# OSU-NLP-Group/saev

Hardware: AMD Instinct MI355X
Metric: activations/sec (train step), d_in=1024 x32 k=32 (higher is better)
Workload: dtype f32 (encoder: fp16 MFMA first pass with a rigorous error margin, survivors recomputed exactly in fp32; all else fp32)

## Files before the change

### saev_amd/csrc/common.h

```cpp
#pragma once
#include <hip/hip_runtime.h>
#include <stdint.h>

#define WAVE 64

typedef float f32x4 __attribute__((ext_vector_type(4)));
typedef float f32x16 __attribute__((ext_vector_type(16)));

__device__ __forceinline__ int32_t f2key(float f) {
    int32_t b = __float_as_int(f);
    return b >= 0 ? b : (b ^ 0x7fffffff);
}
__device__ __forceinline__ float key2f(int32_t k) {
    return __int_as_float(k >= 0 ? k : (k ^ 0x7fffffff));
}
__device__ __forceinline__ uint32_t f2ukey(float f) {
    uint32_t b = __float_as_uint(f);
    return (b & 0x80000000u) ? ~b : (b | 0x80000000u);
}
__device__ __forceinline__ float ukey2f(uint32_t k) {
    return __uint_as_float((k & 0x80000000u) ? (k & 0x7fffffffu) : ~k);
}

__device__ __forceinline__ float wave_sum(float v) {
#pragma unroll
    for (int o = 32; o > 0; o >>= 1) v += __shfl_xor(v, o, 64);
    return v;
}
__device__ __forceinline__ double wave_sum_d(double v) {
#pragma unroll
    for (int o = 32; o > 0; o >>= 1) v += __shfl_xor(v, o, 64);
    return v;
}
__device__ __forceinline__ int wave_sum_i(int v) {
#pragma unroll
    for (int o = 32; o > 0; o >>= 1) v += __shfl_xor(v, o, 64);
    return v;
}
__device__ __forceinline__ float wave_max(float v) {
#pragma unroll
    for (int o = 32; o > 0; o >>= 1) v = fmaxf(v, __shfl_xor(v, o, 64));
    return v;
}

#define NEG_INF (-__builtin_huge_valf())

__device__ __forceinline__ float rpg_apply(float g, float sc, float w) { return __builtin_fmaf(-sc, w, g); }
template <int NV>
__device__ __forceinline__ float rpg_row_stats(const f32x4 (&g)[NV], const f32x4 (&w)[NV], int project, float* sc_out) {
    float dot = 0.f, nsq = 0.f;
#pragma unroll
    for (int n = 0; n < NV; ++n)
#pragma unroll
        for (int e = 0; e < 4; ++e) { dot = __builtin_fmaf(g[n][e], w[n][e], dot); nsq = __builtin_fmaf(w[n][e], w[n][e], nsq); }
    dot = wave_sum(dot);
    nsq = wave_sum(nsq);
    const float sc = (project && nsq > 0.f) ? dot / nsq : 0.f;
    float sq = 0.f;
#pragma unroll
    for (int n = 0; n < NV; ++n)
#pragma unroll
        for (int e = 0; e < 4; ++e) { const float t = rpg_apply(g[n][e], sc, w[n][e]); sq = __builtin_fmaf(t, t, sq); }
    *sc_out = sc;
    return wave_sum(sq);
}
```

### saev_amd/csrc/kernels.h

```cpp
#pragma once
#include <hip/hip_runtime.h>
#include <stdint.h>

#include "../../include/saev_amd.h"

enum { EPI_DENSE = 0, EPI_TOPK = 1 };

struct EncodeArgs {
    const float* x;
    const float* W_enc;
    const float* b_enc;
    int n_rows, D, S;
    int s_splits;
    float* h_out;
    int ngroups;
    int32_t* gmax;
    int gmax_stride;
    int32_t* cand_cnt;
    float* cand_val;
    int32_t* cand_idx;
    int cand_cap;
    int cand_stride;
    const int32_t* enable_flag;
    int enable_when;
};

size_t encode_gemm_smem_bytes();
hipError_t launch_encode_gemm(const EncodeArgs& a, int epi, hipStream_t stream);
int encode_gemm_tile_rows();
int encode_gemm_tile_latents();

struct SelectDenseArgs {
    const float* h;
    int n_rows, S;
    int k;
    const int32_t* k_dev;
    const int32_t* mask;
    int32_t* idx_out;
    float* val_out;
    int out_stride;
    const int32_t* enable_flag;
    int enable_when;
};
hipError_t launch_select_dense(const SelectDenseArgs& a, hipStream_t stream);

struct SelectCandArgs {
    const int32_t* cand_cnt;
    const float* cand_val;
    const int32_t* cand_idx;
    int cand_cap, cand_stride, n_rows, k;
    int32_t* idx_out;
    float* val_out;
    int out_stride;
    const int32_t* enable_flag;
    int enable_when;
    const float* row_margin;
    const float* x;
    const float* W_encT;
    const float* b_enc;
    int D;
    int32_t* surv_idx;
    float* surv_val;
    int32_t* surv_cnt;
    int32_t* refine_overflow;
    const int32_t* tau_max;
    int32_t* invalid;
    int32_t* ovf;
    int32_t* surv_rng;
    int lat_range, n_ranges;
    const float* sum_part;
    const float* sum_bias;
    int sum_n;
    size_t sum_plane;
};
hipError_t launch_refine_exact(const SelectCandArgs& a, hipStream_t stream);
constexpr int REFINE_CAP = 512;
constexpr int RS_SLICE = 32;
constexpr int RS_ROWS_MAX = 8;
constexpr int RS_LAT_RANGE = 32768;
constexpr int RS_MAX_RANGES = 8;
struct RefineSlicesArgs {
    const int32_t* surv_idx; const int32_t* surv_cnt; float* surv_val; const int32_t* surv_rng;
    const float* xS; const float* WeS; const float* b_enc; float* part;
    int n_rows, S, D, lat_range, n_ranges;
    const int32_t* enable_flag; int enable_when;
};
hipError_t launch_refine_slices(const RefineSlicesArgs& a, hipStream_t stream);
hipError_t launch_select_cand(const SelectCandArgs& a, hipStream_t stream);
hipError_t launch_init_i32(int32_t* p, int32_t v, int n, hipStream_t stream);
hipError_t launch_encoder_init(int32_t* cand_cnt, int n_rows, int32_t* gmax, int n_gmax, hipStream_t stream,
                               int32_t* tau_max = nullptr, const int32_t* enable_flag = nullptr, int enable_when = 0);
hipError_t launch_pre_encode(int32_t* cand_cnt, int n_rows, int32_t* gmax, int n_gmax, const float* xnorm, int D,
                             const float* wg_part, int n_part, const float* scales, int32_t* pre_flag, float* wmax_prev,
                             float* margin, int32_t* flags1, hipStream_t stream);
hipError_t launch_heur_gate(float* state, const int32_t* pre_flag, int32_t* gate, hipStream_t stream);
hipError_t launch_heur_update(float* state, const int32_t* bad, const float* cand_mean, int k, const int32_t* gate,
                              hipStream_t stream);
hipError_t launch_step_zero(saev_step_stats* stats, float* upper, int32_t* flag0, hipStream_t stream);
hipError_t launch_wnorm_max(const float* W_encT, int S, int D, float* wg_scratch, float* wmax, hipStream_t stream);
hipError_t launch_f16r_scales(const float* xmax_part, int n_part, const float* wmax, float* scales, hipStream_t stream);
hipError_t launch_pow2_scale(const float* absmax, float* pair, hipStream_t stream);
hipError_t launch_center_stats(const float* x, const float* mu, int n, int D, float* xnorm, float* wg_absmax,
                               hipStream_t stream, const float* xmax = nullptr);
hipError_t launch_row_margins(const float* xnorm, int n, int D, const float* wg_part, int n_part, const float* scales,
                              int32_t* pre_flag, float* wmax_prev, float* margin, hipStream_t stream);
hipError_t launch_overflow_check(const int32_t* cand_cnt, int n_rows, int cap, const int32_t* pre_flag,
                                 int32_t* need_dense, int32_t* n_overflow, int32_t* cand_max, hipStream_t stream,
                                 int32_t* dense_out = nullptr, int32_t* run_out = nullptr, float* cand_mean = nullptr,
                                 const int32_t* enable_flag = nullptr, const int32_t* dense_src = nullptr);

struct __attribute__((aligned(8))) RowStats {
    float sse_scaled;
    float l0;
    float l1;
    float aux_sse;
    double sse64;
    double sumsq64;
};

struct DecodeArgs {
    const float* x;
    const int32_t* idx;
    const float* val;
    int code_stride, k;
    const float* W_dec;
    const float* b_dec;
    int n_rows, D, S;
    int idx_limit;
    const float* upper;
    float gscale;
    int training;
    float* g;
    float* x_hat;
    int32_t* fired;
    RowStats* rowstats;
    float* gS;
    float* xS;
    float* dval_out;
    uint32_t* csc_bitmap;
    int csc_words;
};
hipError_t launch_decode(const DecodeArgs& a, hipStream_t stream);
bool decode_forms_dval(int D, int k);
bool decode_matry_forms_dval(int D, int k);

constexpr int MAX_PREFIXES = 16;
struct MatryArgs {
    int P;
    int32_t cuts[MAX_PREFIXES];
    float* G;
    int g_rows_all;
};
hipError_t launch_decode_matry(const DecodeArgs& a, const MatryArgs& m, hipStream_t stream);

struct CscArgs {
    const int32_t* idx;
    int code_stride, k;
    const int32_t* k_dev;
    int n_rows, S;
    uint32_t* bitmap;
    int words;
    int32_t* grp_prefix;
    int32_t* counts;
    int32_t* scan_totals;
    int32_t* starts;
    int2* pairs;
    int32_t* chunk_starts;
    int32_t* part_starts;
    int32_t* work_latent;
    int2* pv;
    int32_t* plat;
    const float* val;
    int2* pv2;
    const float* dval;
    int P;
    int32_t cuts[16];
    int32_t* zero_word;
    int32_t epoch;
};
hipError_t launch_csc_build(const CscArgs& a, hipStream_t stream, bool bitmap_clean = false, const float* colsum_m = nullptr,
                            int colsum_D = 0, long colsum_row_stride = 0, float* colsum_partials = nullptr,
                            float* colsum_out = nullptr, bool prefilled = false);

constexpr int DW_CHUNK = 64;

struct DwRowsArgs {
    const int32_t* starts;
    const int32_t* chunk_starts;
    const int32_t* work_latent;
    const int32_t* part_starts;
    const int2* pairs;
    const float* val;
    const float* W_dec;
    const float* g;
    const float* x;
    int D, S;
    int P;
    int32_t cuts[MAX_PREFIXES];
    const int32_t* k_dev;
    int accumulate;
    float* dW_dec;
    float* dW_encT;
    float* db_enc;
    float* partials;
    float* db_partials;
    int lat_lo, lat_hi;
    int part;
    float* dval;
    float2* row_proj;
    int project;
    float* enc_sq;
    uint32_t* clear_bitmap;
    int clear_words;
};
hipError_t launch_dw_rows(const DwRowsArgs& a, int max_work, hipStream_t stream);

constexpr int DWS_RUN = 64, DWS_SLICE = 32;
constexpr int DWS_FIRST = 1, DWS_LAST = 2, DWS_END = 4;
struct DwSlicesArgs {
    const int32_t* starts;
    const int2* pv;
    int2* pv2;
    const int32_t* plat;
    const float* gS;
    const float* xS;
    const float* W_dec;
    int n_rows, D, S, pair_cap;
    int P;
    float* dvp;
    float* dW_dec;
    float* dW_encT;
// ... 325 lines not shown
```

### saev_amd/csrc/select.hip

```cpp
#include "common.h"
#include "kernels.h"

namespace {

constexpr int SD_THREADS = 256;

__device__ __forceinline__ int block_excl_scan_256(int v, int* lds_wave_tot, int& total) {
    const int lane = threadIdx.x & 63, w = threadIdx.x >> 6;
    int incl = v;
#pragma unroll
    for (int o = 1; o < 64; o <<= 1) {
        int n = __shfl_up(incl, o, 64);
        if (lane >= o) incl += n;
    }
    if (lane == 63) lds_wave_tot[w] = incl;
    __syncthreads();
    int base = 0, tot = 0;
#pragma unroll
    for (int i = 0; i < 4; ++i) {
        const int t = lds_wave_tot[i];
        if (i < w) base += t;
        tot += t;
    }
    total = tot;
// ... 327 lines not shown
        int32_t idx = 0x7fffffff;
        if (p < n) { key = f2ukey(cv[p]); idx = ci[p]; }
        const bool sel = p < n && ((key > T) || (key == T && idx <= idx_cut));
        const unsigned long long m = __ballot(sel);
        const int pos = base + __popcll(m & ((1ull << lane) - 1ull));
        if (sel && pos < 64) { s_idx[w][pos] = idx; s_val[w][pos] = ukey2f(key); }
        base += __popcll(m);
    }
    sort_by_idx_and_store(a, row, k, s_idx[w][lane], s_val[w][lane], lane);
}

__device__ __forceinline__ void select_small_row(const SelectCandArgs& a, int row, int n, const float* cv, const int32_t* ci) {
    const int lane = threadIdx.x & 63;
    const int k = min(a.k, n);
    uint32_t key = 0u;
    int32_t idx = 0x7fffffff;
    if (lane < n) {
        key = f2ukey(cv[lane]);
        idx = ci[lane];
    }
#pragma unroll
    for (int size = 2; size <= 64; size <<= 1) {
#pragma unroll
        for (int stride = size >> 1; stride > 0; stride >>= 1) {
            const uint32_t o_key = __shfl_xor(key, stride, 64);
            const int32_t o_idx = __shfl_xor(idx, stride, 64);
            const bool other_first = (o_key > key) || (o_key == key && o_idx < idx);
            const bool up = ((lane & size) == 0);
            const bool lower = ((lane & stride) == 0);
            const bool take_other = (lower == up) ? other_first : !other_first;
            if (take_other) { key = o_key; idx = o_idx; }
        }
    }
    if (a.tau_max != nullptr) {
        const float kth = ukey2f(__shfl(key, max(k - 1, 0), 64));
        if (lane == 0 && (n < a.k || kth < key2f(a.tau_max[row]))) *a.invalid = 1;
    }
    const bool win = lane < k;
    sort_by_idx_and_store(a, row, k, win ? idx : 0x7fffffff, win ? ukey2f(key) : 0.f, lane);
}

template <bool BIG>
__global__ __launch_bounds__(256) void select_cand_kernel(SelectCandArgs a) {
    if (a.enable_flag != nullptr && (*a.enable_flag != 0) != (a.enable_when != 0)) return;
    __shared__ int32_t s_idx[4][64];
    __shared__ float s_val[4][64];
    const int row = blockIdx.x * 4 + (threadIdx.x >> 6);
    if (row >= a.n_rows) return;
    const int cnt = a.cand_cnt[row];
    if (a.ovf != nullptr && (threadIdx.x & 63) == 0 && cnt > a.cand_cap) atomicOr(&a.ovf[0], 1);
    if (a.ovf != nullptr && a.row_margin != nullptr && (threadIdx.x & 63) == 0 && !(a.row_margin[row] < 3.0e38f)) atomicOr(&a.ovf[0], 1);
    const int n = min(cnt, a.cand_cap);
    const float* cv = a.cand_val + (size_t)row * a.cand_stride;
    const int32_t* ci = a.cand_idx + (size_t)row * a.cand_stride;
    __shared__ float l_sum[4][REFINE_CAP];
    if (a.sum_part != nullptr) {
        float* const lv = l_sum[threadIdx.x >> 6];
        for (int j = threadIdx.x & 63; j < n; j += 64) {
            const size_t o = (size_t)row * a.cand_stride + j;
            float sv = 0.f;
            int c = 0;
            for (; c + 8 <= a.sum_n; c += 8) {
                float v[8];
#pragma unroll
                for (int u = 0; u < 8; ++u) v[u] = a.sum_part[(size_t)(c + u) * a.sum_plane + o];
#pragma unroll
                for (int u = 0; u < 8; ++u) sv += v[u];
            }
            for (; c < a.sum_n; ++c) sv += a.sum_part[(size_t)c * a.sum_plane + o];
            lv[j] = sv + a.sum_bias[ci[j]];
        }
        __asm__ volatile("" ::: "memory");
        cv = lv;
    }
    if (n <= 64 && a.row_margin == nullptr) select_small_row(a, row, n, cv, ci);
    else if (n <= 512) select_cand_row<8>(a, row, n, s_idx, s_val, cv, ci);
    else if (n <= 1024) select_cand_row<16>(a, row, n, s_idx, s_val, cv, ci);
    else if (n <= 2048) select_cand_row<32>(a, row, n, s_idx, s_val, cv, ci);
    else if constexpr (BIG) select_cand_row<64>(a, row, n, s_idx, s_val, cv, ci);
    else select_cand_row_stream(a, row, n, s_idx, s_val, cv, ci);
}

__global__ void init_i32_kernel(int32_t* p, int32_t v, int n) {
    const int i = blockIdx.x * blockDim.x + threadIdx.x;
    if (i < n) p[i] = v;
}

__global__ void encoder_init_kernel(int32_t* cand_cnt, int n_rows, int32_t* gmax, int n_gmax, int32_t* tau_max,
                                    const int32_t* enable_flag, int enable_when) {
    if (enable_flag != nullptr && (*enable_flag != 0) != (enable_when != 0)) return;
    const int i = blockIdx.x * blockDim.x + threadIdx.x;
    if (i < n_rows) cand_cnt[i] = 0;
    if (i < n_gmax) gmax[i] = INT32_MIN;
    if (tau_max != nullptr && i < n_rows) tau_max[i] = INT32_MIN;
}
__global__ void step_zero_kernel(saev_step_stats* stats, float* upper, int32_t* flag0) {
    if (threadIdx.x == 0) {
        *stats = saev_step_stats{};
        *upper = 0.f;
        *flag0 = 0;
    }
}

template <int NV>
__global__ __launch_bounds__(256) void refine_exact_kernel(SelectCandArgs a) {
    if (a.enable_flag != nullptr && (*a.enable_flag != 0) != (a.enable_when != 0)) return;
    const int lane = threadIdx.x & 63;
    const int row = blockIdx.x * 4 + (threadIdx.x >> 6);
    if (row >= a.n_rows) return;
    const int ns = a.surv_cnt[row];
    const int D4 = a.D >> 2;
    f32x4 xv[NV];
    const f32x4* xr = reinterpret_cast<const f32x4*>(a.x + (size_t)row * a.D);
#pragma unroll
    for (int n = 0; n < NV; ++n) xv[n] = (lane + 64 * n < D4) ? xr[lane + 64 * n] : f32x4{0.f, 0.f, 0.f, 0.f};
    const int32_t* si = a.surv_idx + (size_t)row * REFINE_CAP;
    float* sv = a.surv_val + (size_t)row * REFINE_CAP;
    for (int j0 = 0; j0 < ns; j0 += 8) {
        const int32_t my = si[min(j0 + (lane & 7), ns - 1)];
        float p[8];
#pragma unroll
        for (int t = 0; t < 8; ++t) {
            const int32_t li = __shfl(my, t, 64);
            const f32x4* wr = reinterpret_cast<const f32x4*>(a.W_encT + (size_t)li * a.D);
            float acc = 0.f;
#pragma unroll
            for (int n = 0; n < NV; ++n) {
                if (lane + 64 * n < D4) {
                    const f32x4 wv = wr[lane + 64 * n];
                    acc += xv[n][0] * wv[0] + xv[n][1] * wv[1] + xv[n][2] * wv[2] + xv[n][3] * wv[3];
                }
            }
            p[t] = acc;
        }
        const float r = wave_reduce_scatter8(p, lane);
        if ((lane & 7) == 0) {
            const int t = lane >> 3;
            if (j0 + t < ns) sv[j0 + t] = r + a.b_enc[si[j0 + t]];
        }
    }
}

typedef int i32x4 __attribute__((ext_vector_type(4)));
__device__ __forceinline__ f32x4 rs_buf_load16(__amdgpu_buffer_rsrc_t r, uint32_t voff) {
    const i32x4 v = __builtin_amdgcn_raw_buffer_load_b128(r, voff, 0, 0);
    return f32x4{__int_as_float(v[0]), __int_as_float(v[1]), __int_as_float(v[2]), __int_as_float(v[3])};
}
__device__ __forceinline__ float group8_reduce_scatter(float (&p)[8], int li) {
    {
        const bool up = (li & 4) != 0;
#pragma unroll
        for (int i = 0; i < 4; ++i) {
            const float keep = up ? p[i + 4] : p[i], send = up ? p[i] : p[i + 4];
            p[i] = keep + __shfl_xor(send, 4, 64);
        }
    }
    {
        const bool up = (li & 2) != 0;
#pragma unroll
        for (int i = 0; i < 2; ++i) {
            const float keep = up ? p[i + 2] : p[i], send = up ? p[i] : p[i + 2];
            p[i] = keep + __shfl_xor(send, 2, 64);
        }
    }
    const bool up = (li & 1) != 0;
    const float keep = up ? p[1] : p[0], send = up ? p[0] : p[1];
    return keep + __shfl_xor(send, 1, 64);
}
#ifndef RS_BATCHES
#define RS_BATCHES 2
#endif
template <int RS_ROWS>
__global__ __launch_bounds__(256) void refine_slices_kernel(RefineSlicesArgs a, int wg_per_combo) {
    if (a.enable_flag != nullptr && (*a.enable_flag != 0) != (a.enable_when != 0)) return;
    const int lane = threadIdx.x & 63, gi = lane >> 3, li = lane & 7;
    const int xcd = blockIdx.x & 7, q = blockIdx.x >> 3;
    const int combo = q / wg_per_combo;
    const int slice = xcd + 8 * (combo / a.n_ranges), range = combo % a.n_ranges;
    if (slice * RS_SLICE >= a.D) return;
    const int wgi = q % wg_per_combo;
    const int lat_lo = range * a.lat_range, lat_hi = min(a.S, lat_lo + a.lat_range);
    const int sel = (lane & 56) << 2;
    const __amdgpu_buffer_rsrc_t wres = __builtin_amdgcn_make_buffer_rsrc(
        const_cast<float*>(a.WeS) + (size_t)slice * a.S * RS_SLICE, 0, (uint32_t)a.S * 128u, 0x00020000);
    const f32x4* const xs = reinterpret_cast<const f32x4*>(a.xS + (size_t)slice * a.n_rows * RS_SLICE);
    float* const part = a.part + (size_t)slice * a.n_rows * REFINE_CAP;
    const uint32_t li16 = (uint32_t)li * 16u;
    const int row0 = (wgi * RS_ROWS * 4 + (int)(threadIdx.x >> 6)) * 8 + gi;
    int jb[RS_ROWS], je[RS_ROWS];
    f32x4 xr[RS_ROWS];
#pragma unroll
    for (int t = 0; t < RS_ROWS; ++t) {
        const int row = row0 + 32 * t;
        const bool rok = row < a.n_rows;
        je[t] = rok ? a.surv_rng[(size_t)row * RS_MAX_RANGES + range] : 0;
        jb[t] = (rok && range > 0) ? a.surv_rng[(size_t)row * RS_MAX_RANGES + range - 1] : 0;
        xr[t] = rok ? xs[(size_t)row * 8 + li] : f32x4{0.f, 0.f, 0.f, 0.f};
    }
    int t = 0, j0 = jb[0], j_end = je[0];
    f32x4 x4 = xr[0];
    auto advance = [&]() {
#pragma unroll
        for (int s = 1; s < RS_ROWS; ++s) {
            const bool adv = j0 >= j_end && t == s - 1;
            t = adv ? s : t;
            j0 = adv ? jb[s] : j0;
            j_end = adv ? je[s] : j_end;
#pragma unroll
            for (int e = 0; e < 4; ++e) x4[e] = adv ? xr[s][e] : x4[e];
        }
    };
    advance();
#pragma unroll 1
    while (__any(j0 < j_end)) {
        const int row = row0 + 32 * t;
        int32_t my[RS_BATCHES];
        bool mine[RS_BATCHES];
        f32x4 w[RS_BATCHES][8];
#pragma unroll
        for (int h = 0; h < RS_BATCHES; ++h) {
            my[h] = (j0 + 8 * h + li < j_end) ? a.surv_idx[(size_t)row * REFINE_CAP + j0 + 8 * h + li] : -1;
            mine[h] = my[h] >= lat_lo && my[h] < lat_hi;
        }
#pragma unroll
        for (int h = 0; h < RS_BATCHES; ++h) {
            const uint32_t off_my = mine[h] ? (uint32_t)my[h] * 128u : 0xFFFFFF00u;
#pragma unroll
            for (int u = 0; u < 8; ++u) {
                const uint32_t off = (uint32_t)__builtin_amdgcn_ds_bpermute(sel + 4 * u, (int)off_my);
                w[h][u] = rs_buf_load16(wres, off | li16);
            }
        }
#pragma unroll
        for (int h = 0; h < RS_BATCHES; ++h) {
            float p[8];
#pragma unroll
            for (int u = 0; u < 8; ++u) p[u] = x4[0] * w[h][u][0] + x4[1] * w[h][u][1] + x4[2] * w[h][u][2] + x4[3] * w[h][u][3];
            const float r = group8_reduce_scatter(p, li);
            if (mine[h]) part[(size_t)row * REFINE_CAP + j0 + 8 * h + li] = r;
        }
        j0 += 8 * RS_BATCHES;
        advance();
    }
}

__global__ __launch_bounds__(256) void rownorm_wgmax_kernel(const float* m, int R, int D, float* wg_max) {
    __shared__ float sh[4];
    const int lane = threadIdx.x & 63, w = threadIdx.x >> 6;
    const int r = blockIdx.x * 4 + w;
    float s = 0.f;
    if (r < R) {
        const f32x4* p = reinterpret_cast<const f32x4*>(m + (size_t)r * D);
        for (int q = lane; q < (D >> 2); q += 64) {
            const f32x4 v = p[q];
            s += v[0] * v[0] + v[1] * v[1] + v[2] * v[2] + v[3] * v[3];
        }
        s = wave_sum(s);
    }
    if (lane == 0) sh[w] = sqrtf(s);
    __syncthreads();
    if (threadIdx.x == 0) wg_max[blockIdx.x] = fmaxf(fmaxf(sh[0], sh[1]), fmaxf(sh[2], sh[3]));
}
__global__ __launch_bounds__(1024) void max_reduce_kernel(const float* v, int n, float* out) {
    __shared__ float sh[16];
    float m = 0.f;
    for (int i = threadIdx.x; i < n; i += 1024) m = fmaxf(m, v[i]);
    m = wave_max(m);
    if ((threadIdx.x & 63) == 0) sh[threadIdx.x >> 6] = m;
    __syncthreads();
    if (threadIdx.x == 0) {
        float t = 0.f;
        for (int i = 0; i < 16; ++i) t = fmaxf(t, sh[i]);
        *out = t;
    }
}
__device__ __forceinline__ float round_f16_sig(float v) {
    const uint32_t b = __float_as_uint(v);
    return __uint_as_float((b + 0x0FFFu + ((b >> 13) & 1u)) & 0xFFFFE000u);
}
__global__ __launch_bounds__(256) void center_stats_kernel(const float* x, const float* mu, int n, int D,
                                                           float* xnorm, float* wg_max, const float* xmax) {
    __shared__ float sh[4];
    const int lane = threadIdx.x & 63, w = threadIdx.x >> 6;
    const int r = blockIdx.x * 4 + w;
    float s = 0.f, m = 0.f, sd = 0.f;
    const float up = xmax != nullptr ? *xmax : 1.0f;
    const float back = (up > 0.f && up < 3.0e38f) ? up : 1.0f, inv = 1.0f / back;
    if (r < n) {
        const f32x4* p = reinterpret_cast<const f32x4*>(x + (size_t)r * D);
        const f32x4* mu4 = reinterpret_cast<const f32x4*>(mu);
        const int nq = D >> 2;
        for (int q0 = lane; q0 < nq; q0 += 256) {
            f32x4 v[4];
#pragma unroll
            for (int u = 0; u < 4; ++u) {
                const int q = q0 + 64 * u;
                v[u] = q < nq ? p[q] - mu4[q] : f32x4{0.f, 0.f, 0.f, 0.f};
            }
#pragma unroll
            for (int u = 0; u < 4; ++u) {
                m = fmaxf(fmaxf(fmaxf(m, fabsf(v[u][0])), fabsf(v[u][1])), fmaxf(fabsf(v[u][2]), fabsf(v[u][3])));
                f32x4 d;
#pragma unroll
                for (int e = 0; e < 4; ++e) d[e] = (v[u][e] - round_f16_sig(v[u][e])) * inv;
                v[u] = v[u] * inv;
                s += v[u][0] * v[u][0] + v[u][1] * v[u][1] + v[u][2] * v[u][2] + v[u][3] * v[u][3];
                sd += d[0] * d[0] + d[1] * d[1] + d[2] * d[2] + d[3] * d[3];
            }
        }
        s = wave_sum(s);
        sd = wave_sum(sd);
        if (lane == 0) { xnorm[2 * r] = back * sqrtf(s); xnorm[2 * r + 1] = back * sqrtf(sd) * 1.000001f; }
    }
    m = wave_max(m);
    if (lane == 0) sh[w] = m;
    __syncthreads();
    if (threadIdx.x == 0) wg_max[blockIdx.x] = fmaxf(fmaxf(sh[0], sh[1]), fmaxf(sh[2], sh[3]));
}
__device__ __forceinline__ float f16r_margin(float xnorm_row, float xdelta_row, float wmax, float dwmax, float bmax, int D, float x_scale) {
    const float rnd = 1.02f * (xdelta_row * wmax + xnorm_row * dwmax + xdelta_row * dwmax);
    const float acc = (1.05f * (float)D * 2.384185791015625e-07f + 7.62939453125e-06f) * xnorm_row * wmax;
    const float sub = sqrtf((float)D) * 6.103515625e-05f / x_scale * wmax;
    const float m = 2.0f * (rnd + acc + sub) + 2.0f * 1.1920929e-07f * bmax;
    return m == m ? m : __builtin_inff();
}
__device__ __forceinline__ bool f16r_scale_ok(float wmax, float w_scale) {
    const float t = wmax * w_scale;
    return t < 60000.0f && (t >= 2048.0f || wmax == 0.f);
}
__global__ __launch_bounds__(256) void row_margin_kernel(const float* xnorm, int n, int D, const float* wg_part, int n_part,
                                                         const float* scales, int32_t* pre_flag, float* wmax_prev,
                                                         float* margin) {
    __shared__ float sh[3][4];
    float bm = 0.f, wm = 0.f, dm = 0.f;
    for (int i = threadIdx.x; i < n_part; i += 256) { bm = fmaxf(bm, wg_part[i]); wm = fmaxf(wm, wg_part[n_part + i]); dm = fmaxf(dm, wg_part[2 * n_part + i]); }
    bm = wave_max(bm); wm = wave_max(wm); dm = wave_max(dm);
    if ((threadIdx.x & 63) == 0) { sh[0][threadIdx.x >> 6] = bm; sh[1][threadIdx.x >> 6] = wm; sh[2][threadIdx.x >> 6] = dm; }
    __syncthreads();
    const float bmax = fmaxf(fmaxf(sh[0][0], sh[0][1]), fmaxf(sh[0][2], sh[0][3]));
    const float wmax = fmaxf(fmaxf(sh[1][0], sh[1][1]), fmaxf(sh[1][2], sh[1][3]));
    const float dwmax = fmaxf(fmaxf(sh[2][0], sh[2][1]), fmaxf(sh[2][2], sh[2][3]));
    if (blockIdx.x == 0 && threadIdx.x == 0) {
        if (!f16r_scale_ok(wmax, scales[1])) *pre_flag = 1;
        *wmax_prev = wmax;
    }
    const int r = blockIdx.x * 256 + threadIdx.x;
    if (r >= n) return;
    margin[r] = f16r_margin(xnorm[2 * r], xnorm[2 * r + 1], wmax, dwmax, bmax, D, scales[0]);
}
__global__ __launch_bounds__(256) void pre_encode_kernel(int32_t* cand_cnt, int n_rows, int32_t* gmax, int n_gmax,
                                                         const float* xnorm, int D, const float* wg_part, int n_part,
                                                         const float* scales, int32_t* pre_flag, float* wmax_prev,
                                                         float* margin, int32_t* flags1) {
    const int i = blockIdx.x * 256 + threadIdx.x;
    if (i < n_rows) cand_cnt[i] = 0;
    if (i < n_gmax) gmax[i] = INT32_MIN;
    if (xnorm == nullptr) {
        if (i == 0) { flags1[0] = (pre_flag != nullptr && *pre_flag != 0) ? 1 : 0; flags1[1] = 0; flags1[2] = 0; }
        return;
    }
    if ((int)blockIdx.x * 256 >= n_rows && blockIdx.x != 0) return;
    __shared__ float sh[3][4];
    float bm = 0.f, wm = 0.f, dm = 0.f;
    for (int j = threadIdx.x; j < n_part; j += 256) { bm = fmaxf(bm, wg_part[j]); wm = fmaxf(wm, wg_part[n_part + j]); dm = fmaxf(dm, wg_part[2 * n_part + j]); }
    bm = wave_max(bm); wm = wave_max(wm); dm = wave_max(dm);
    if ((threadIdx.x & 63) == 0) { sh[0][threadIdx.x >> 6] = bm; sh[1][threadIdx.x >> 6] = wm; sh[2][threadIdx.x >> 6] = dm; }
    __syncthreads();
    const float bmax = fmaxf(fmaxf(sh[0][0], sh[0][1]), fmaxf(sh[0][2], sh[0][3]));
    const float wmax = fmaxf(fmaxf(sh[1][0], sh[1][1]), fmaxf(sh[1][2], sh[1][3]));
    const float dwmax = fmaxf(fmaxf(sh[2][0], sh[2][1]), fmaxf(sh[2][2], sh[2][3]));
    if (i == 0) {
        int pre = *pre_flag != 0 ? 1 : 0;
        if (!f16r_scale_ok(wmax, scales[1])) { pre = 1; *pre_flag = 1; }
        *wmax_prev = wmax;
        flags1[0] = pre; flags1[1] = 0; flags1[2] = 0;
    }
    if (i >= n_rows) return;
    margin[i] = f16r_margin(xnorm[2 * i], xnorm[2 * i + 1], wmax, dwmax, bmax, D, scales[0]);
}
__global__ __launch_bounds__(256) void pre_encode2_kernel(PreEncode2Args a) {
    __shared__ float sh[5][4];
    const int i = blockIdx.x * 256 + threadIdx.x;
    if ((int)blockIdx.x >= a.nb_rows) {
        const int d = ((int)blockIdx.x - a.nb_rows) * 256 + threadIdx.x;
        if (d >= a.D || !a.update_mu) return;
        float t = 0.f;
        int b = 0;
        for (; b + 8 <= a.n_rowblk; b += 8) {
            float v[8];
#pragma unroll
            for (int u = 0; u < 8; ++u) v[u] = a.col_part[(size_t)(b + u) * a.D + d];
#pragma unroll
            for (int u = 0; u < 8; ++u) t += v[u];
        }
        for (; b < a.n_rowblk; ++b) t += a.col_part[(size_t)b * a.D + d];
// ... 107 lines not shown
    __syncthreads();
    int c = 0, m = 0, t = 0;
    for (int i = threadIdx.x; i < n_rows; i += blockDim.x) { const int v = cand_cnt[i]; c += (v > cap); m = max(m, v); t += min(v, cap); }
    c = wave_sum_i(c);
    t = wave_sum_i(t);
#pragma unroll
    for (int o = 32; o > 0; o >>= 1) m = max(m, __shfl_xor(m, o, 64));
    if ((threadIdx.x & 63) == 0) { if (c) atomicAdd(&sh, c); atomicMax(&shmax, m); atomicAdd(&shsum, t); }
    __syncthreads();
    if (threadIdx.x == 0) {
        const int pre = (pre_flag && *pre_flag) ? 1 : 0;
        *n_overflow = sh;
        *cand_max = shmax;
        if (cand_mean != nullptr) *cand_mean = (float)shsum / (float)max(n_rows, 1);
        if (run_out == nullptr) {
            *bad_out = (pre || sh > 0) ? 1 : 0;
            if (dense_out != nullptr) *dense_out = dense_src != nullptr ? (*dense_src != 0 ? 1 : 0) : pre;
        } else {
            const int dense = (*dense_out != 0 || sh > 0) ? 1 : 0;
            *dense_out = dense;
            *run_out = dense ? 0 : 1;
        }
    }
}

__global__ void heur_gate_kernel(float* state, const int32_t* pre_flag, int32_t* gate) {
    if (threadIdx.x != 0) return;
    int g = (pre_flag != nullptr && *pre_flag != 0) ? 1 : 0;
    if (state[5] > 0.f) { state[5] -= 1.f; g = 1; }
    *gate = g;
}
__global__ void heur_update_kernel(float* state, const int32_t* bad, const float* cand_mean, int k, const int32_t* gate) {
    if (threadIdx.x != 0 || *gate != 0) return;
    float z = state[0];
    state[2] += 1.f;
    if (*bad != 0) {
        z -= 0.3f;
        state[1] += 1.f;
        state[4] += 1.f;
        if (state[4] >= 3.f) { state[4] = 0.f; state[5] = 256.f; z = 1.5f; }
    } else {
        state[4] = 0.f;
        if (*cand_mean > 3.f * (float)k) z += 0.002f;
    }
    state[0] = fminf(fmaxf(z, 0.5f), 3.5f);
}

}

hipError_t launch_select_dense(const SelectDenseArgs& a, hipStream_t stream) {
    if (a.n_rows <= 0) return hipSuccess;
    hipLaunchKernelGGL(select_dense_kernel, dim3(a.n_rows), dim3(SD_THREADS), 0, stream, a);
    return hipGetLastError();
}

hipError_t launch_select_cand(const SelectCandArgs& a, hipStream_t stream) {
    if (a.n_rows <= 0) return hipSuccess;
    if (a.cand_cap > 4096 || (a.sum_part != nullptr && a.cand_cap > REFINE_CAP)) return hipErrorInvalidValue;
    if (a.k > 32) hipLaunchKernelGGL(select_cand_kernel<true>, dim3((a.n_rows + 3) / 4), dim3(256), 0, stream, a);
    else hipLaunchKernelGGL(select_cand_kernel<false>, dim3((a.n_rows + 3) / 4), dim3(256), 0, stream, a);
    return hipGetLastError();
}

hipError_t launch_init_i32(int32_t* p, int32_t v, int n, hipStream_t stream) {
    if (n <= 0) return hipSuccess;
    hipLaunchKernelGGL(init_i32_kernel, dim3((n + 255) / 256), dim3(256), 0, stream, p, v, n);
    return hipGetLastError();
}

hipError_t launch_encoder_init(int32_t* cand_cnt, int n_rows, int32_t* gmax, int n_gmax, hipStream_t stream, int32_t* tau_max,
                               const int32_t* enable_flag, int enable_when) {
    const int n = n_rows > n_gmax ? n_rows : n_gmax;
    if (n <= 0) return hipSuccess;
    hipLaunchKernelGGL(encoder_init_kernel, dim3((n + 255) / 256), dim3(256), 0, stream, cand_cnt, n_rows, gmax, n_gmax, tau_max,
                       enable_flag, enable_when);
    return hipGetLastError();
}
hipError_t launch_pre_encode(int32_t* cand_cnt, int n_rows, int32_t* gmax, int n_gmax, const float* xnorm, int D,
                             const float* wg_part, int n_part, const float* scales, int32_t* pre_flag, float* wmax_prev,
                             float* margin, int32_t* flags1, hipStream_t stream) {
    const int n = std::max(1, n_rows > n_gmax ? n_rows : n_gmax);
    hipLaunchKernelGGL(pre_encode_kernel, dim3((n + 255) / 256), dim3(256), 0, stream, cand_cnt, n_rows, gmax, n_gmax, xnorm, D,
                       wg_part, n_part, scales, pre_flag, wmax_prev, margin, flags1);
    return hipGetLastError();
}
hipError_t launch_follower_scales(const float* xside, const float* wmax, float* scales, int32_t* pre_flag, int keep_w, hipStream_t stream) {
    hipLaunchKernelGGL(follower_scales_kernel, dim3(1), dim3(64), 0, stream, xside, wmax, scales, pre_flag, keep_w);
    return hipGetLastError();
}
hipError_t launch_pre_encode2(PreEncode2Args a, hipStream_t stream) {
    a.nb_rows = (std::max(1, std::max(a.n_rows, a.n_gmax)) + 255) / 256;
    hipLaunchKernelGGL(pre_encode2_kernel, dim3(a.nb_rows + (a.D + 255) / 256), dim3(256), 0, stream, a);
    return hipGetLastError();
}
hipError_t launch_heur_gate(float* state, const int32_t* pre_flag, int32_t* gate, hipStream_t stream) {
    hipLaunchKernelGGL(heur_gate_kernel, dim3(1), dim3(64), 0, stream, state, pre_flag, gate);
    return hipGetLastError();
}
hipError_t launch_heur_update(float* state, const int32_t* bad, const float* cand_mean, int k, const int32_t* gate,
                              hipStream_t stream) {
    hipLaunchKernelGGL(heur_update_kernel, dim3(1), dim3(64), 0, stream, state, bad, cand_mean, k, gate);
    return hipGetLastError();
}
hipError_t launch_step_zero(saev_step_stats* stats, float* upper, int32_t* flag0, hipStream_t stream) {
    hipLaunchKernelGGL(step_zero_kernel, dim3(1), dim3(64), 0, stream, stats, upper, flag0);
    return hipGetLastError();
}

hipError_t launch_wnorm_max(const float* W_encT, int S, int D, float* wg_scratch, float* wmax, hipStream_t stream) {
    const int nwg = (S + 3) / 4;
    hipLaunchKernelGGL(rownorm_wgmax_kernel, dim3(nwg), dim3(256), 0, stream, W_encT, S, D, wg_scratch);
    hipLaunchKernelGGL(max_reduce_kernel, dim3(1), dim3(1024), 0, stream, wg_scratch, nwg, wmax);
    return hipGetLastError();
}
hipError_t launch_f16r_scales(const float* xmax_part, int n_part, const float* wmax, float* scales, hipStream_t stream) {
    hipLaunchKernelGGL(f16r_scales_kernel, dim3(1), dim3(256), 0, stream, xmax_part, n_part, wmax, scales);
    return hipGetLastError();
}
hipError_t launch_pow2_scale(const float* absmax, float* pair, hipStream_t stream) {
    hipLaunchKernelGGL(pow2_scale_kernel, dim3(1), dim3(64), 0, stream, absmax, pair);
    return hipGetLastError();
}
hipError_t launch_center_stats(const float* x, const float* mu, int n, int D, float* xnorm, float* wg_absmax,
                               hipStream_t stream, const float* xmax) {
    hipLaunchKernelGGL(center_stats_kernel, dim3((n + 3) / 4), dim3(256), 0, stream, x, mu, n, D, xnorm, wg_absmax, xmax);
    return hipGetLastError();
}
hipError_t launch_max_reduce(const float* v, int n, float* out, hipStream_t stream) {
    hipLaunchKernelGGL(max_reduce_kernel, dim3(1), dim3(1024), 0, stream, v, n, out);
    return hipGetLastError();
}
hipError_t launch_row_margins(const float* xnorm, int n, int D, const float* wg_part, int n_part, const float* scales,
                              int32_t* pre_flag, float* wmax_prev, float* margin, hipStream_t stream) {
    hipLaunchKernelGGL(row_margin_kernel, dim3((n + 255) / 256), dim3(256), 0, stream, xnorm, n, D, wg_part, n_part, scales,
                       pre_flag, wmax_prev, margin);
    return hipGetLastError();
}

hipError_t launch_refine_exact(const SelectCandArgs& a, hipStream_t stream) {
    if (a.n_rows <= 0) return hipSuccess;
    const dim3 grid((a.n_rows + 3) / 4), block(256);
    const int nv = (a.D / 4 + 63) / 64;
#define RF(N) hipLaunchKernelGGL(refine_exact_kernel<N>, grid, block, 0, stream, a)
    if (nv <= 1) RF(1); else if (nv <= 2) RF(2); else if (nv <= 3) RF(3); else if (nv <= 4) RF(4);
    else if (nv <= 6) RF(6); else if (nv <= 8) RF(8); else if (nv <= 12) RF(12); else if (nv <= 16) RF(16);
    else return hipErrorInvalidValue;
#undef RF
    return hipGetLastError();
}

hipError_t launch_refine_slices(const RefineSlicesArgs& a, hipStream_t stream) {
    if (a.n_rows <= 0) return hipSuccess;
    if (a.D % RS_SLICE != 0 || (uint64_t)a.S * 128ull >= (1ull << 32) - 256ull || a.n_ranges <= 0) return hipErrorInvalidValue;
    const int rows = a.n_rows >= 8192 ? RS_ROWS_MAX : 4;
    const int wg_per_combo = (a.n_rows + 32 * rows - 1) / (32 * rows);
    const int slice_blocks = (a.D / RS_SLICE + 7) / 8;
    const dim3 grid(8 * slice_blocks * a.n_ranges * wg_per_combo);
    if (rows == 4) hipLaunchKernelGGL(refine_slices_kernel<4>, grid, dim3(256), 0, stream, a, wg_per_combo);
    else hipLaunchKernelGGL(refine_slices_kernel<RS_ROWS_MAX>, grid, dim3(256), 0, stream, a, wg_per_combo);
    return hipGetLastError();
}

hipError_t launch_overflow_check(const int32_t* cand_cnt, int n_rows, int cap, const int32_t* pre_flag,
                                 int32_t* need_dense, int32_t* n_overflow, int32_t* cand_max, hipStream_t stream,
                                 int32_t* dense_out, int32_t* run_out, float* cand_mean, const int32_t* enable_flag,
                                 const int32_t* dense_src) {
    hipLaunchKernelGGL(overflow_check_kernel, dim3(1), dim3(1024), 0, stream, cand_cnt, n_rows, cap, pre_flag,
                       need_dense, n_overflow, cand_max, dense_out, run_out, cand_mean, enable_flag, dense_src);
    return hipGetLastError();
}
```

Baseline: 6.243 million.

## Use DPP lane exchange, prefetch survivor indices, shrink rows per block in refine_slices

In the sliced exact-refine kernel, the ds_bpermute index broadcast and the shfl_xor reductions are replaced with DPP moves, which avoid LDS-based cross-lane traffic. Survivor indices are now read through buffer loads and prefetched one iteration ahead, so their latency overlaps the dot-product and reduction work. Results are written with buffer stores. The large-batch configuration drops from 8 rows per thread group to 1, which gives more blocks and less per-thread row-selection state but less reuse per block.

```diff
diff --git a/saev_amd/csrc/common.h b/saev_amd/csrc/common.h
--- a/saev_amd/csrc/common.h
+++ b/saev_amd/csrc/common.h
@@ -45,6 +45,19 @@
 
 #define NEG_INF (-__builtin_huge_valf())
 
+__device__ __forceinline__ int group8_xor4(int v) {
+    const int t = __builtin_amdgcn_update_dpp(v, v, 0x104, 0xF, 0x5, false);
+    return __builtin_amdgcn_update_dpp(t, v, 0x114, 0xF, 0xA, false);
+}
+template <bool HI>
+__device__ __forceinline__ int group8_quad_copy(int v) {
+    return HI ? __builtin_amdgcn_update_dpp(v, v, 0x104, 0xF, 0x5, false) : __builtin_amdgcn_update_dpp(v, v, 0x114, 0xF, 0xA, false);
+}
+template <int U>
+__device__ __forceinline__ int quad_bcast(int v) {
+    return __builtin_amdgcn_mov_dpp(v, (U & 3) * 0x55, 0xF, 0xF, true);
+}
+
 __device__ __forceinline__ float rpg_apply(float g, float sc, float w) { return __builtin_fmaf(-sc, w, g); }
 template <int NV>
 __device__ __forceinline__ float rpg_row_stats(const f32x4 (&g)[NV], const f32x4 (&w)[NV], int project, float* sc_out) {
diff --git a/saev_amd/csrc/kernels.h b/saev_amd/csrc/kernels.h
--- a/saev_amd/csrc/kernels.h
+++ b/saev_amd/csrc/kernels.h
@@ -76,7 +76,7 @@
 hipError_t launch_refine_exact(const SelectCandArgs& a, hipStream_t stream);
 constexpr int REFINE_CAP = 512;
 constexpr int RS_SLICE = 32;
-constexpr int RS_ROWS_MAX = 8;
+constexpr int RS_ROWS_BIG = 1;
 constexpr int RS_LAT_RANGE = 32768;
 constexpr int RS_MAX_RANGES = 8;
 struct RefineSlicesArgs {
diff --git a/saev_amd/csrc/select.hip b/saev_amd/csrc/select.hip
--- a/saev_amd/csrc/select.hip
+++ b/saev_amd/csrc/select.hip
@@ -503,7 +503,7 @@
 #pragma unroll
         for (int i = 0; i < 4; ++i) {
             const float keep = up ? p[i + 4] : p[i], send = up ? p[i] : p[i + 4];
-            p[i] = keep + __shfl_xor(send, 4, 64);
+            p[i] = keep + __int_as_float(group8_xor4(__float_as_int(send)));
         }
     }
     {
@@ -511,12 +511,12 @@
 #pragma unroll
         for (int i = 0; i < 2; ++i) {
             const float keep = up ? p[i + 2] : p[i], send = up ? p[i] : p[i + 2];
-            p[i] = keep + __shfl_xor(send, 2, 64);
+            p[i] = keep + __int_as_float(__builtin_amdgcn_mov_dpp(__float_as_int(send), 0x4E, 0xF, 0xF, true));
         }
     }
     const bool up = (li & 1) != 0;
     const float keep = up ? p[1] : p[0], send = up ? p[0] : p[1];
-    return keep + __shfl_xor(send, 1, 64);
+    return keep + __int_as_float(__builtin_amdgcn_mov_dpp(__float_as_int(send), 0xB1, 0xF, 0xF, true));
 }
 #ifndef RS_BATCHES
 #define RS_BATCHES 2
@@ -531,7 +531,6 @@
     if (slice * RS_SLICE >= a.D) return;
     const int wgi = q % wg_per_combo;
     const int lat_lo = range * a.lat_range, lat_hi = min(a.S, lat_lo + a.lat_range);
-    const int sel = (lane & 56) << 2;
     const __amdgpu_buffer_rsrc_t wres = __builtin_amdgcn_make_buffer_rsrc(
         const_cast<float*>(a.WeS) + (size_t)slice * a.S * RS_SLICE, 0, (uint32_t)a.S * 128u, 0x00020000);
     const f32x4* const xs = reinterpret_cast<const f32x4*>(a.xS + (size_t)slice * a.n_rows * RS_SLICE);
@@ -557,41 +556,61 @@
             t = adv ? s : t;
             j0 = adv ? jb[s] : j0;
             j_end = adv ? je[s] : j_end;
-#pragma unroll
-            for (int e = 0; e < 4; ++e) x4[e] = adv ? xr[s][e] : x4[e];
-        }
+        }
+    };
+    auto take_x = [&]() {
+#pragma unroll
+        for (int s = 1; s < RS_ROWS; ++s)
+#pragma unroll
+            for (int e = 0; e < 4; ++e) x4[e] = t == s ? xr[s][e] : x4[e];
     };
     advance();
+    take_x();
+    const __amdgpu_buffer_rsrc_t ires = __builtin_amdgcn_make_buffer_rsrc(const_cast<int32_t*>(a.surv_idx), 0,
+                                                                         (uint32_t)a.n_rows * (uint32_t)(REFINE_CAP * 4), 0x00020000);
+    const __amdgpu_buffer_rsrc_t pres = __builtin_amdgcn_make_buffer_rsrc(part, 0, (uint32_t)a.n_rows * (uint32_t)(REFINE_CAP * 4), 0x00020000);
+    auto load_idx = [&](int32_t (&my)[RS_BATCHES], bool (&ok)[RS_BATCHES]) {
+        const int o = (row0 + 32 * t) * REFINE_CAP + j0 + li;
+#pragma unroll
+        for (int h = 0; h < RS_BATCHES; ++h) {
+            ok[h] = j0 + 8 * h + li < j_end;
+            my[h] = __builtin_amdgcn_raw_buffer_load_b32(ires, ok[h] ? (uint32_t)(o + 8 * h) * 4u : 0xFFFFFF00u, 0, 0);
+        }
+    };
+    int32_t my_n[RS_BATCHES];
+    bool ok_n[RS_BATCHES];
+    load_idx(my_n, ok_n);
 #pragma unroll 1
     while (__any(j0 < j_end)) {
-        const int row = row0 + 32 * t;
-        int32_t my[RS_BATCHES];
+        const int po = (row0 + 32 * t) * REFINE_CAP + j0 + li;
         bool mine[RS_BATCHES];
         f32x4 w[RS_BATCHES][8];
 #pragma unroll
         for (int h = 0; h < RS_BATCHES; ++h) {
-            my[h] = (j0 + 8 * h + li < j_end) ? a.surv_idx[(size_t)row * REFINE_CAP + j0 + 8 * h + li] : -1;
-            mine[h] = my[h] >= lat_lo && my[h] < lat_hi;
-        }
-#pragma unroll
-        for (int h = 0; h < RS_BATCHES; ++h) {
-            const uint32_t off_my = mine[h] ? (uint32_t)my[h] * 128u : 0xFFFFFF00u;
-#pragma unroll
-            for (int u = 0; u < 8; ++u) {
-                const uint32_t off = (uint32_t)__builtin_amdgcn_ds_bpermute(sel + 4 * u, (int)off_my);
-                w[h][u] = rs_buf_load16(wres, off | li16);
-            }
-        }
+            mine[h] = ok_n[h] && my_n[h] >= lat_lo && my_n[h] < lat_hi;
+            const int off_my = (int)(mine[h] ? (uint32_t)my_n[h] * 128u : 0xFFFFFF00u);
+            const int off_lo = group8_quad_copy<false>(off_my), off_hi = group8_quad_copy<true>(off_my);
+            w[h][0] = rs_buf_load16(wres, (uint32_t)quad_bcast<0>(off_lo) | li16);
+            w[h][1] = rs_buf_load16(wres, (uint32_t)quad_bcast<1>(off_lo) | li16);
+            w[h][2] = rs_buf_load16(wres, (uint32_t)quad_bcast<2>(off_lo) | li16);
+            w[h][3] = rs_buf_load16(wres, (uint32_t)quad_bcast<3>(off_lo) | li16);
+            w[h][4] = rs_buf_load16(wres, (uint32_t)quad_bcast<0>(off_hi) | li16);
+            w[h][5] = rs_buf_load16(wres, (uint32_t)quad_bcast<1>(off_hi) | li16);
+            w[h][6] = rs_buf_load16(wres, (uint32_t)quad_bcast<2>(off_hi) | li16);
+            w[h][7] = rs_buf_load16(wres, (uint32_t)quad_bcast<3>(off_hi) | li16);
+        }
+        j0 += 8 * RS_BATCHES;
+        advance();
+        load_idx(my_n, ok_n);
 #pragma unroll
         for (int h = 0; h < RS_BATCHES; ++h) {
             float p[8];
 #pragma unroll
             for (int u = 0; u < 8; ++u) p[u] = x4[0] * w[h][u][0] + x4[1] * w[h][u][1] + x4[2] * w[h][u][2] + x4[3] * w[h][u][3];
             const float r = group8_reduce_scatter(p, li);
-            if (mine[h]) part[(size_t)row * REFINE_CAP + j0 + 8 * h + li] = r;
-        }
-        j0 += 8 * RS_BATCHES;
-        advance();
+            if (mine[h]) __builtin_amdgcn_raw_buffer_store_b32(__float_as_int(r), pres, (uint32_t)(po + 8 * h) * 4u, 0, 0);
+        }
+        take_x();
     }
 }
 
@@ -1005,12 +1024,12 @@
 hipError_t launch_refine_slices(const RefineSlicesArgs& a, hipStream_t stream) {
     if (a.n_rows <= 0) return hipSuccess;
     if (a.D % RS_SLICE != 0 || (uint64_t)a.S * 128ull >= (1ull << 32) - 256ull || a.n_ranges <= 0) return hipErrorInvalidValue;
-    const int rows = a.n_rows >= 8192 ? RS_ROWS_MAX : 4;
+    const int rows = a.n_rows >= 8192 ? RS_ROWS_BIG : 4;
     const int wg_per_combo = (a.n_rows + 32 * rows - 1) / (32 * rows);
     const int slice_blocks = (a.D / RS_SLICE + 7) / 8;
     const dim3 grid(8 * slice_blocks * a.n_ranges * wg_per_combo);
     if (rows == 4) hipLaunchKernelGGL(refine_slices_kernel<4>, grid, dim3(256), 0, stream, a, wg_per_combo);
-    else hipLaunchKernelGGL(refine_slices_kernel<RS_ROWS_MAX>, grid, dim3(256), 0, stream, a, wg_per_combo);
+    else hipLaunchKernelGGL(refine_slices_kernel<RS_ROWS_BIG>, grid, dim3(256), 0, stream, a, wg_per_combo);
     return hipGetLastError();
 }
 
```

Result: no change. 6.285 million (median of 6 runs) (+0.7%).
